# Artemarius/cuda-gaussian-splatting

Hardware: AMD Instinct MI355X
Metric: fwd+bwd Mpixels/s @1080p, 1M Gaussians, SH3 (higher is better)
Workload: dtype f32

## Files before the change

cuda-gaussian-splatting_amd/csrc/cugs_common.h:

```cpp
#pragma once

#include <hip/hip_runtime.h>
#include <stdint.h>

#include "../../include/cugs_hip.h"
#include "../../include/cugs_detmath.h"

#ifndef CUGS_BLOCK
#define CUGS_BLOCK 256
#endif
#define CUGS_WAVE 64

#define CUGS_RETURN_IF_HIP(expr)                    \
    do {                                            \
        hipError_t _e = (expr);                     \
        if (_e != hipSuccess) return (int)_e;       \
    } while (0)

#define CUGS_LAUNCH_CHECK() CUGS_RETURN_IF_HIP(hipGetLastError())

static inline bool cugs_aligned16(const void* p) { return (reinterpret_cast<uintptr_t>(p) & 15u) == 0; }

typedef float cugs_v4f __attribute__((ext_vector_type(4)));
typedef float cugs_v2f __attribute__((ext_vector_type(2)));
// ... 7 lines not shown
    __builtin_nontemporal_store(t, reinterpret_cast<cugs_v4f*>(p));
}
__device__ __forceinline__ void cugs_stnt(float* p, float v) { __builtin_nontemporal_store(v, p); }

struct CamArgs {
    float view[16];
    float fx, fy, cx, cy;
    int width, height;
    float cc[3];
    float log_mod;
};

static inline CamArgs cugs_make_cam_args(const cugs_camera* c, float scale_modifier) {
    CamArgs a;
    for (int i = 0; i < 16; ++i) a.view[i] = c->view[i];
    a.fx = c->fx; a.fy = c->fy; a.cx = c->cx; a.cy = c->cy;
    a.width = c->width; a.height = c->height;
    a.cc[0] = c->cam_center[0]; a.cc[1] = c->cam_center[1]; a.cc[2] = c->cam_center[2];
    a.log_mod = logf(scale_modifier + 1e-8f);
    return a;
}

int cugs_sort_key_slots(void* workspace, size_t bytes, int64_t n, int width, int height, uint32_t** keys, int4** rect,
                        uint32_t** prect, uint32_t** range_flag, uint32_t** zero, uint32_t* nzero)
    __attribute__((visibility("hidden")));

__device__ __forceinline__ unsigned cugs_xcd_remap(unsigned bid, unsigned nwg) {
    unsigned xcd = bid & 7u, q = nwg >> 3, r = nwg & 7u;
    unsigned base = (xcd < r) ? xcd * (q + 1u) : r * (q + 1u) + (xcd - r) * q;
    return base + (bid >> 3);
}

#ifndef CUGS_ROW_GROUP
#define CUGS_ROW_GROUP 2
#endif
__device__ __forceinline__ unsigned cugs_blend_tile(unsigned bid, unsigned ntx, unsigned nty) {
    const unsigned lin = cugs_xcd_remap(bid, ntx * nty);
#if CUGS_ROW_GROUP == 0
    return lin;
#else
    constexpr unsigned G = CUGS_ROW_GROUP;
    unsigned row = lin / ntx;
    const unsigned col = lin - row * ntx;
    const unsigned nunits = (nty + G - 1u) / G;
    unsigned c = 0, urow = row;
#pragma unroll
    for (unsigned k = 0; k < 7u; ++k) {
// ... 10 lines not shown
```

cuda-gaussian-splatting_amd/csrc/cugs_gaussian_math.h:

```cpp
#pragma once

#include "cugs_common.h"

struct V3 { float x, y, z; };
struct Sym2 { float a, b, c; };
struct Sym3 { float xx, xy, xz, yy, yz, zz; };
struct M3 { float m00, m01, m02, m10, m11, m12, m20, m21, m22; };
struct M23 { float r0x, r0y, r0z, r1x, r1y, r1z; };

struct GradMoments { float m1x, m1y, m2xx, m2xy, m2yy; };
struct Grad2D { float mx, my, a, b, c; };
__device__ __forceinline__ Grad2D grads_from_moments(const GradMoments& m, float a, float b, float c) {
    Grad2D g;
    g.mx = a * m.m1x + b * m.m1y;
    g.my = b * m.m1x + c * m.m1y;
    g.a = -0.5f * m.m2xx;
    g.b = -m.m2xy;
    g.c = -0.5f * m.m2yy;
    return g;
}

__device__ __forceinline__ M3 view_rotation(const CamArgs& c) {
    return M3{c.view[0], c.view[1], c.view[2], c.view[4], c.view[5], c.view[6],
              c.view[8], c.view[9], c.view[10]};
// ... 150 lines not shown
    *out_of_range = false;
    if (three_pass) {
        const uint32_t off = key - CUGS_DEPTH_KEY_BASE;
        const bool emits = tiles > 0 && w > 0;
        *out_of_range = emits && !(off >= 1u && off < CUGS_DEPTH_KEY_SPAN);
        key = emits ? min(off, CUGS_DEPTH_KEY_SPAN - 1u) : 0u;
    }
    return SortRecord{key, make_int4(x0, y0, w | (h << 16), tiles > 0 ? tiles : 0)};
}

constexpr int CUGS_PRECT_MAX_TILES = 127;
__host__ __device__ inline bool cugs_prect_packable(int ntx, int nty) { return ntx <= CUGS_PRECT_MAX_TILES && nty <= CUGS_PRECT_MAX_TILES; }
__device__ __forceinline__ uint32_t pack_rect(int4 r) {
    const int w = r.z & 0xFFFF, h = r.z >> 16;
    if (w == 0) return 0x80000000u | (uint32_t)r.w;
    return (uint32_t)r.x | ((uint32_t)r.y << 7) | ((uint32_t)w << 14) | ((uint32_t)h << 21);
}
__device__ __forceinline__ int4 unpack_rect(uint32_t v) {
    if (v & 0x80000000u) return make_int4(0, 0, 0, (int)(v & 0x7FFFFFFFu));
    const int x0 = (int)(v & 127u), y0 = (int)((v >> 7) & 127u), w = (int)((v >> 14) & 127u), h = (int)((v >> 21) & 127u);
    return make_int4(x0, y0, w | (h << 16), w * h);
}

__device__ __forceinline__ V3 view_direction(V3 p, const CamArgs& c) {
    float dx = p.x - c.cc[0], dy = p.y - c.cc[1], dz = p.z - c.cc[2];
    float nrm = fmaxf(sqrtf(dx * dx + dy * dy + dz * dz), 1e-8f);
    return V3{dx / nrm, dy / nrm, dz / nrm};
}

__device__ __forceinline__ void sh_basis(int degree, V3 d, float (&Y)[16]) {
    const float x = d.x, y = d.y, z = d.z;
    Y[0] = 0.28209479177387814f;
    if (degree >= 1) {
        Y[1] = -0.4886025119029199f * y;
        Y[2] = 0.4886025119029199f * z;
        Y[3] = -0.4886025119029199f * x;
    }
    if (degree >= 2) {
        const float xx = x * x, yy = y * y, zz = z * z;
        Y[4] = 1.0925484305920792f * (x * y);
        Y[5] = 1.0925484305920792f * (y * z);
        Y[6] = 0.31539156525252005f * (2 * zz - xx - yy);
        Y[7] = 1.0925484305920792f * (x * z);
        Y[8] = 0.5462742152960396f * (xx - yy);
    }
    if (degree >= 3) {
// ... 58 lines not shown
```

cuda-gaussian-splatting_amd/csrc/project_forward.hip:

```cpp
#include "cugs_gaussian_math.h"

namespace {

template <int C>
struct ShTile {
    static constexpr int ROW = 3 * C;
    static constexpr int LROW = (ROW % 2 == 0) ? ROW + 1 : ROW;
};

template <int C, bool ALIGNED>
__device__ __forceinline__ void stage_sh_rows(const float* __restrict__ sh, int64_t base, int count,
                                              float* s_sh) {
    constexpr int ROW = ShTile<C>::ROW, LROW = ShTile<C>::LROW;
    const float* src = sh + base * ROW;
    const int total = count * ROW;
    const int tid = threadIdx.x;
    if (ALIGNED && count == CUGS_BLOCK) {
        constexpr int TOTAL4 = CUGS_BLOCK * ROW / 4, PER = (TOTAL4 + CUGS_BLOCK - 1) / CUGS_BLOCK;
        const float4* src4 = reinterpret_cast<const float4*>(src);
        float4 v[PER];
#pragma unroll
        for (int i = 0; i < PER; ++i) {
            const int e4 = tid + i * CUGS_BLOCK;
            v[i] = (e4 < TOTAL4) ? cugs_ldnt(src4 + e4) : make_float4(0.f, 0.f, 0.f, 0.f);
// ... 23 lines not shown
#pragma unroll
            for (int k = 0; k < 4; ++k) {
                s_sh[row * LROW + col] = vals[k];
                if (++col == ROW) { col = 0; ++row; }
            }
        }
        for (int e = (total4 << 2) + tid; e < total; e += CUGS_BLOCK) {
            int row = e / ROW, col = e - row * ROW;
            s_sh[row * LROW + col] = src[e];
        }
    } else {
        for (int e = tid; e < total; e += CUGS_BLOCK) {
            int row = e / ROW, col = e - row * ROW;
            s_sh[row * LROW + col] = src[e];
        }
    }
}

struct ProjPtrs {
    const float* positions; const float* rotations; const float* scales; const float* opacities;
    const float* sh;
    float* means_2d; float* depths; float* cov_2d_inv; int32_t* radii; int32_t* tiles_touched;
    float* opacities_act; float* rgb; float* packed; uint8_t* colour_gate;
    uint32_t* sort_keys; int4* sort_rect; uint32_t* sort_prect; uint32_t* sort_range_flag;
    uint32_t* sort_zero; uint32_t sort_nzero;
};

template <int C, bool ALIGNED, int PART>
__global__ __launch_bounds__(CUGS_BLOCK) void k_project_forward(int64_t n, int degree, CamArgs cam,
                                                                ProjPtrs p) {
    constexpr int LROW = ShTile<C>::LROW;
    constexpr int OUT_F = 6 * CUGS_BLOCK + CUGS_PACKED_STRIDE * CUGS_BLOCK;
    constexpr int SH_F = (PART == 1) ? 0 : CUGS_BLOCK * LROW;
    __shared__ __attribute__((aligned(16))) float s_sh[SH_F > OUT_F ? SH_F : OUT_F];

    const int64_t base = (int64_t)blockIdx.x * CUGS_BLOCK;
    const int count = (int)min((int64_t)CUGS_BLOCK, n - base);
    for (uint32_t z = blockIdx.x * CUGS_BLOCK + threadIdx.x; z < p.sort_nzero; z += gridDim.x * CUGS_BLOCK) p.sort_zero[z] = 0u;
    const int64_t idx = base + threadIdx.x;
    const bool live = idx < n;
    const int64_t ld = live ? idx : (n - 1);
    const V3 pos{cugs_ldnt(p.positions + ld * 3 + 0), cugs_ldnt(p.positions + ld * 3 + 1), cugs_ldnt(p.positions + ld * 3 + 2)};
    float in_opa = 0.0f, in_s0 = 0.0f, in_s1 = 0.0f, in_s2 = 0.0f;
    float4 q = make_float4(1.0f, 0.0f, 0.0f, 0.0f);
    {
        in_opa = cugs_ldnt(p.opacities + ld);
        in_s0 = cugs_ldnt(p.scales + ld * 3 + 0); in_s1 = cugs_ldnt(p.scales + ld * 3 + 1); in_s2 = cugs_ldnt(p.scales + ld * 3 + 2);
// ... 46 lines not shown
        const Sym3 S = gram(scale_columns(qr.R, s));
        const Jac J = jacobian(t, cam.fx, cam.fy);
        const Sym2 cov = screen_covariance(project_matrix_full(J, W), S);
        Sym2 inv_c;
        const float det = invert_sym2(cov, inv_c);
        if (det > 0.0f) {
            inv = inv_c;
            int r = splat_radius(cov);
            if (r > 0) {
                r = min(r, max(cam.width, cam.height));
                radius = r;
                const int ntx = (cam.width + CUGS_TILE - 1) / CUGS_TILE;
                const int nty = (cam.height + CUGS_TILE - 1) / CUGS_TILE;
                tr = tile_rect_of(mx, my, r, cam.width, cam.height, ntx, nty);
                tiles = max((tr.x1 - tr.x0) * (tr.y1 - tr.y0), 0);
            }
        }
    }

    p.depths[idx] = depth;
    p.radii[idx] = radius;
    p.tiles_touched[idx] = tiles;
    p.opacities_act[idx] = opa;
    if (p.sort_keys) {
        bool bad;
        const SortRecord rec = sort_record_of(depth, tiles, radius, tr, true, &bad);
        if (bad) atomicOr(p.sort_range_flag, 1u);
        p.sort_keys[idx] = rec.key;
        if (p.sort_prect) p.sort_prect[idx] = pack_rect(rec.rect);
        else p.sort_rect[idx] = rec.rect;
    }
    if (ALIGNED && count == CUGS_BLOCK && p.packed) {
        reinterpret_cast<float2*>(p.means_2d)[idx] = make_float2(mx, my);
        if constexpr (PART == 0) __syncthreads();
        float* s_rgb = s_sh;
        float* s_cov = s_sh + 3 * CUGS_BLOCK;
        float4* s_pk = reinterpret_cast<float4*>(s_sh + 6 * CUGS_BLOCK);
        const int t = threadIdx.x;
        s_rgb[t * 3 + 0] = col[0]; s_rgb[t * 3 + 1] = col[1]; s_rgb[t * 3 + 2] = col[2];
        s_cov[t * 3 + 0] = inv.a; s_cov[t * 3 + 1] = inv.b; s_cov[t * 3 + 2] = inv.c;
        const float tau = (opa >= (1.0f / 255.0f)) ? logf(255.0f * opa) : -1.0f;
        s_pk[t * 3 + 0] = make_float4(mx, my, inv.a, inv.b);
        s_pk[t * 3 + 1] = make_float4(inv.c, opa, tau, 0.0f);
        s_pk[t * 3 + 2] = make_float4(col[0], 0.0f, col[1], col[2]);
        __syncthreads();
        if (t < 3 * CUGS_BLOCK / 4) {
            if constexpr (PART == 0) reinterpret_cast<float4*>(p.rgb + base * 3)[t] = reinterpret_cast<const float4*>(s_rgb)[t];
            reinterpret_cast<float4*>(p.cov_2d_inv + base * 3)[t] = reinterpret_cast<const float4*>(s_cov)[t];
        }
        float4* g_pk = reinterpret_cast<float4*>(p.packed + base * CUGS_PACKED_STRIDE);
        if constexpr (PART == 0) {
#pragma unroll
            for (int k = 0; k < 3; ++k) g_pk[t + k * CUGS_BLOCK] = s_pk[t + k * CUGS_BLOCK];
// ... 174 lines not shown
                                    const float* positions, const float* rotations,
                                    const float* scales, const float* opacities,
                                    const float* sh_coeffs, const cugs_camera* camera_host,
                                    float scale_modifier, float* means_2d, float* depths,
                                    float* cov_2d_inv, int32_t* radii, int32_t* tiles_touched,
                                    float* opacities_act, float* rgb, float* packed, uint8_t* colour_gate,
                                    void* sort_workspace, size_t sort_workspace_bytes, void* stream) {
    if (n < 0 || !camera_host) return CUGS_EINVAL;
    if (active_degree < 0 || active_degree > 3) return CUGS_EINVAL;
    if ((active_degree + 1) * (active_degree + 1) > num_coeffs) return CUGS_EINVAL;
    if (num_coeffs != 1 && num_coeffs != 4 && num_coeffs != 9 && num_coeffs != 16) return CUGS_EINVAL;
    if (n == 0) return 0;
    if (!positions || !rotations || !scales || !opacities || !sh_coeffs || !means_2d || !depths ||
        !cov_2d_inv || !radii || !tiles_touched || !opacities_act || !rgb)
        return CUGS_EINVAL;
    if (packed && !cugs_aligned16(packed)) return CUGS_EALIGN;
    if (n > (int64_t)2147483647) return CUGS_EOVERFLOW;

    const CamArgs cam = cugs_make_cam_args(camera_host, scale_modifier);
    ProjPtrs p{positions, rotations, scales, opacities, sh_coeffs, means_2d, depths, cov_2d_inv,
               radii, tiles_touched, opacities_act, rgb, packed, colour_gate, nullptr, nullptr, nullptr, nullptr, nullptr, 0u};
    if (sort_workspace) {
        int rc = cugs_sort_key_slots(sort_workspace, sort_workspace_bytes, n, camera_host->width, camera_host->height,
                                     &p.sort_keys, &p.sort_rect, &p.sort_prect, &p.sort_range_flag, &p.sort_zero, &p.sort_nzero);
        if (rc) return rc;
    }
    const bool aligned = cugs_aligned16(sh_coeffs) && cugs_aligned16(rotations) && cugs_aligned16(rgb) &&
                         cugs_aligned16(cov_2d_inv) && (reinterpret_cast<uintptr_t>(means_2d) & 7u) == 0;
    hipStream_t st = static_cast<hipStream_t>(stream);
    switch (num_coeffs) {
        case 1: return launch_project<1>(n, active_degree, cam, p, aligned, st);
        case 4: return launch_project<4>(n, active_degree, cam, p, aligned, st);
        case 9: return launch_project<9>(n, active_degree, cam, p, aligned, st);
        default: return launch_project<16>(n, active_degree, cam, p, aligned, st);
    }
}
}

extern "C" int cugs_project_forward(int64_t n, int num_coeffs, int active_degree,
                                    const float* positions, const float* rotations,
                                    const float* scales, const float* opacities,
                                    const float* sh_coeffs, const cugs_camera* camera_host,
                                    float scale_modifier, float* means_2d, float* depths,
                                    float* cov_2d_inv, int32_t* radii, int32_t* tiles_touched,
                                    float* opacities_act, float* rgb, float* packed, uint8_t* colour_gate,
                                    void* stream) {
    return project_forward_impl(n, num_coeffs, active_degree, positions, rotations, scales, opacities, sh_coeffs,
// ... 13 lines not shown
    return project_forward_impl(n, num_coeffs, active_degree, positions, rotations, scales, opacities, sh_coeffs,
                                camera_host, scale_modifier, means_2d, depths, cov_2d_inv, radii, tiles_touched,
                                opacities_act, rgb, packed, colour_gate, sort_workspace, sort_workspace_bytes, stream);
}

extern "C" int cugs_project_forward_geometry(int64_t n, const float* positions, const float* rotations,
                                             const float* scales, const float* opacities,
                                             const cugs_camera* camera_host, float scale_modifier, float* means_2d,
                                             float* depths, float* cov_2d_inv, int32_t* radii, int32_t* tiles_touched,
                                             float* opacities_act, float* packed, void* sort_workspace,
                                             size_t sort_workspace_bytes, void* stream) {
    if (n < 0 || !camera_host) return CUGS_EINVAL;
    if (n == 0) return 0;
    if (!positions || !rotations || !scales || !opacities || !means_2d || !depths || !cov_2d_inv || !radii ||
        !tiles_touched || !opacities_act)
        return CUGS_EINVAL;
    if (packed && !cugs_aligned16(packed)) return CUGS_EALIGN;
    if (n > (int64_t)2147483647) return CUGS_EOVERFLOW;
    const CamArgs cam = cugs_make_cam_args(camera_host, scale_modifier);
    ProjPtrs p{positions, rotations, scales, opacities, nullptr, means_2d, depths, cov_2d_inv, radii, tiles_touched,
               opacities_act, nullptr, packed, nullptr, nullptr, nullptr, nullptr, nullptr, nullptr, 0u};
    if (sort_workspace) {
        int rc = cugs_sort_key_slots(sort_workspace, sort_workspace_bytes, n, camera_host->width, camera_host->height,
                                     &p.sort_keys, &p.sort_rect, &p.sort_prect, &p.sort_range_flag, &p.sort_zero, &p.sort_nzero);
        if (rc) return rc;
    }
    const bool aligned = cugs_aligned16(rotations) && cugs_aligned16(cov_2d_inv) &&
                         (reinterpret_cast<uintptr_t>(means_2d) & 7u) == 0;
    return launch_project<1, 1>(n, 0, cam, p, aligned, static_cast<hipStream_t>(stream));
}

extern "C" int cugs_project_forward_colour(int64_t n, int num_coeffs, int active_degree, const float* positions,
                                           const float* sh_coeffs, const cugs_camera* camera_host, float* rgb,
                                           float* packed, uint8_t* colour_gate, void* stream) {
    if (n < 0 || !camera_host) return CUGS_EINVAL;
    if (active_degree < 0 || active_degree > 3) return CUGS_EINVAL;
    if ((active_degree + 1) * (active_degree + 1) > num_coeffs) return CUGS_EINVAL;
    if (num_coeffs != 1 && num_coeffs != 4 && num_coeffs != 9 && num_coeffs != 16) return CUGS_EINVAL;
    if (n == 0) return 0;
    if (!positions || !sh_coeffs || !rgb) return CUGS_EINVAL;
    if (packed && !cugs_aligned16(packed)) return CUGS_EALIGN;
    if (n > (int64_t)2147483647) return CUGS_EOVERFLOW;
    const CamArgs cam = cugs_make_cam_args(camera_host, 1.0f);
    ProjPtrs p{positions, nullptr, nullptr, nullptr, sh_coeffs, nullptr, nullptr, nullptr, nullptr, nullptr, nullptr, rgb,
               packed, colour_gate, nullptr, nullptr, nullptr, nullptr, nullptr, 0u};
    const bool aligned = cugs_aligned16(sh_coeffs) && cugs_aligned16(rgb);
    hipStream_t st = static_cast<hipStream_t>(stream);
// ... 47 lines not shown
```

cuda-gaussian-splatting_amd/csrc/sort.hip:

```cpp
#include "sort_workspace.h"
#include "sort_radix.h"
#include "sort_emit.h"
#include "sort_tile_order.h"
#include "sort_bin.h"

namespace {

int queue_count(const SortPlan& plan, const SortWsN& ws, const float* means_2d, const float* depths, const int32_t* radii,
                const int32_t* tiles_touched, hipStream_t st, unsigned long long* total_mapped) {
    const uint32_t un = plan.n;
    const int ntx = plan.ntx, nty = plan.nty;
    const bool narrow = plan.depth == DepthRoute::Narrow, direct = plan.route == PairRoute::Direct;
    uint32_t* const range_flag = &ws.ctl->range_flag;
    uint32_t* const q12 = &ws.ctl->q12_count;
    const uint32_t* const ridden = plan.riding ? ws.prect[1] : nullptr;
    int rc;
    if (plan.keys == KeySource::Built) {
        hipLaunchKernelGGL(k_depth_keys_rect, dim3(nblocks_for(un, CUGS_BLOCK)), dim3(CUGS_BLOCK), 0, st, un, depths,
                           means_2d, radii, tiles_touched, plan.width, plan.height, ntx, nty, ws.dkey[narrow ? 0 : 1], ws.rect[0],
                           narrow ? range_flag : static_cast<uint32_t*>(nullptr), ws.sup, plan.depth_clear);
        CUGS_LAUNCH_CHECK();
    }
    uint32_t* sp[SUP_TABLES];
    for (int t = 0; t < SUP_TABLES; ++t) sp[t] = ws.sup + (size_t)t * plan.depth_table;
    if (narrow) {
        uint32_t* const* pr = ws.prect;
        const bool riding = plan.riding;
        if ((rc = radix_pass<uint32_t, true, 1024, CHUNK_DEPTH, RADIX_DEPTH>(ws.dkey[0], nullptr, un, nullptr, 0, DEPTH_BITS, ws.hist, sp[0], ws.tot, ws.dkey[1], ws.dval[1], nullptr, st, riding ? pr[0] : nullptr, pr[1]))) return rc;
        if ((rc = radix_pass<uint32_t, false, 1024, CHUNK_DEPTH, RADIX_DEPTH>(ws.dkey[1], ws.dval[1], un, nullptr, DEPTH_BITS, DEPTH_BITS, ws.hist, sp[1], ws.tot, ws.dkey[0], ws.dval[0], nullptr, st, riding ? pr[1] : nullptr, pr[0]))) return rc;
        if ((rc = radix_pass<uint32_t, false, 1024, CHUNK_DEPTH, RADIX_DEPTH>(ws.dkey[0], ws.dval[0], un, nullptr, 2 * DEPTH_BITS, DEPTH_BITS, ws.hist, sp[2], ws.tot, ws.dkey[1], ws.dval[1], direct ? q12 : nullptr, st, riding ? pr[0] : nullptr, pr[1]))) return rc;
    } else {
        if ((rc = radix_pass<uint32_t, true, 1024, CHUNK_MIN>(ws.dkey[1], nullptr, un, nullptr, 0, 8, ws.hist, sp[0], ws.tot, ws.dkey[0], ws.dval[0], nullptr, st))) return rc;
        if ((rc = radix_pass<uint32_t, false, 1024, CHUNK_MIN>(ws.dkey[0], ws.dval[0], un, nullptr, 8, 8, ws.hist, sp[1], ws.tot, ws.dkey[1], ws.dval[1], nullptr, st))) return rc;
        if ((rc = radix_pass<uint32_t, false, 1024, CHUNK_MIN>(ws.dkey[1], ws.dval[1], un, nullptr, 16, 8, ws.hist, sp[2], ws.tot, ws.dkey[0], ws.dval[0], nullptr, st))) return rc;
        if ((rc = radix_pass<uint32_t, false, 1024, CHUNK_MIN>(ws.dkey[0], ws.dval[0], un, nullptr, 24, 8, ws.hist, sp[3], ws.tot, ws.dkey[1], ws.dval[1], nullptr, st))) return rc;
    }
    if (direct) {
        const uint32_t tiles = (uint32_t)plan.tiles, rows = bin_rows(un);
        hipLaunchKernelGGL(k_bin_count, dim3(rows), dim3(BIN_NT), 0, st, un, BIN_GROUP, ws.dval[1], ws.rect[0], ridden,
                           plan.riding ? static_cast<uint32_t*>(nullptr) : ws.prect[1], (uint32_t)ntx, (uint32_t)nty, ws.bin_table, q12,
                           ws.bin_win);
        CUGS_LAUNCH_CHECK();
        hipLaunchKernelGGL(k_bin_scan, dim3((tiles + CUGS_WAVE - 1) / CUGS_WAVE), dim3(BIN_NT), 0, st, rows, tiles, ws.bin_table,
                           ws.bin_ttot, ws.bin_tpre, ws.bin_csum, q12, range_flag, &ws.ctl->snap_q12,
                           bin_windows(ntx, nty) <= BIN_WINDOWS_MAX ? ws.bin_win : nullptr,
                           (uint32_t)ntx, bin_window_cols(ntx), bin_window_groups(ntx));
        CUGS_LAUNCH_CHECK();
        return 0;
    }
    const uint32_t nfill = nblocks_for(un, FILL_CHUNK);
    hipLaunchKernelGGL(k_fill_blocksums, dim3(nfill), dim3(CUGS_BLOCK), 0, st, un, ws.dval[1], ws.rect[0], ws.rect[1],
                       ws.blocksum, ridden);
    CUGS_LAUNCH_CHECK();
// ... 74 lines not shown
        const int shift = p * per;
        const int b = (bits - shift) < per ? (bits - shift) : per;
        uint32_t* vout = (p == npass - 1) ? vals_final : tv[cur ^ 1];
        rc = radix_pass<K, false, 512, CHUNK_PAIR>(tk[cur], tv[cur], up, dev_count, shift, b, wp.hist, wp.sup + sup_off[p], ws.tot,
                                                   tk[cur ^ 1], vout, p == 0 ? ctl : nullptr, st);
        if (rc) return rc;
        cur ^= 1;
    }
    hipLaunchKernelGGL((k_tile_ranges<K, false>), dim3(nblocks_for(up, CUGS_BLOCK * 8)), dim3(CUGS_BLOCK), 0, st, up, dev_count, tk[cur],
                       (uint32_t)ntx, values_sorted, depths, tile_ranges, keys_sorted, ctl + 1);
    CUGS_LAUNCH_CHECK();
    return 0;
}

template <typename... A>
int sort_pairs_dispatch(const SortPlan& plan, A... args) {
    if (plan.wide_ids) return sort_pairs_typed<uint32_t>(plan, args...);
    return sort_pairs_typed<uint16_t>(plan, args...);
}

}

int cugs_sort_key_slots(void* workspace, size_t bytes, int64_t n, int width, int height, uint32_t** keys, int4** rect,
                        uint32_t** prect, uint32_t** range_flag, uint32_t** zero, uint32_t* nzero) {
    if (!workspace || n < 0 || n > 2147483647ll || width < 0 || height < 0) return CUGS_EINVAL;
    if ((width + CUGS_TILE - 1) / CUGS_TILE > 32767 || (height + CUGS_TILE - 1) / CUGS_TILE > 32767) return CUGS_EOVERFLOW;
    SortWsN ws = carve_n(workspace, n);
    if (bytes < ws.bytes) return CUGS_EWORKSPACE;
    const SortPlan plan = make_sort_plan(n, width, height, 0, KeySource::Prekeyed, DepthRoute::Narrow, PairCount::Predicted);
    *keys = ws.dkey[0];
    *rect = plan.riding ? nullptr : ws.rect[0];
    *prect = plan.riding ? ws.prect[0] : nullptr;
    *range_flag = &ws.ctl->range_flag;
    *zero = ws.sup;
    *nzero = plan.depth_clear;
    return 0;
}

extern "C" size_t cugs_sort_workspace_bytes(int64_t n) {
    if (n < 0) return 0;
    return carve_n(nullptr, n).bytes;
}

extern "C" size_t cugs_sort_pair_workspace_bytes(int64_t total_pairs) {
    if (total_pairs < 0) return 0;
    return carve_p(nullptr, total_pairs).bytes;
}

namespace {
int sort_count_pairs_impl(int64_t n, const float* means_2d, const float* depths,
                                     const int32_t* radii, const int32_t* tiles_touched, int width,
                                     int height, void* workspace, size_t workspace_bytes,
                                     int64_t* total_pairs_host, void* stream, DepthRoute depth) {
    if (n < 0 || width < 0 || height < 0 || !total_pairs_host) return CUGS_EINVAL;
    *total_pairs_host = 0;
// ... 220 lines not shown
```

cuda-gaussian-splatting_amd/csrc/sort_radix.h:

```cpp
#pragma once

#include "sort_workspace.h"

namespace {

__device__ __forceinline__ uint32_t wave_inclusive_scan(uint32_t v) {
    const int lane = threadIdx.x & 63;
#pragma unroll
    for (int d = 1; d < 64; d <<= 1) {
        uint32_t t = __shfl_up(v, d);
        if (lane >= d) v += t;
    }
    return v;
}

template <int NW = 4>
__device__ __forceinline__ uint32_t block_exclusive_scan(uint32_t v, uint32_t* s_tmp, uint32_t* total) {
    const int lane = threadIdx.x & 63, wave = threadIdx.x >> 6;
    uint32_t inc = wave_inclusive_scan(v);
    if (lane == 63) s_tmp[wave] = inc;
    __syncthreads();
    uint32_t base = 0, sum = 0;
#pragma unroll
    for (int w = 0; w < NW; ++w) {
// ... 249 lines not shown
__global__ __launch_bounds__(CUGS_BLOCK) void k_probe_lds_order(uint32_t* __restrict__ violations) {
    __shared__ uint32_t cnt[4][RADIX];
    const uint32_t wave = threadIdx.x >> 6, lane = threadIdx.x & 63, set = blockIdx.x;
    for (uint32_t i = threadIdx.x; i < 4 * RADIX; i += CUGS_BLOCK) (&cnt[0][0])[i] = 0;
    __syncthreads();
    uint32_t d[8], got[8];
#pragma unroll
    for (int r = 0; r < 8; ++r) d[r] = probe_digit(set, wave, r, lane);
#pragma unroll
    for (int r = 0; r < 8; ++r) got[r] = atomicAdd(&cnt[wave][d[r]], 1u);
    uint32_t bad = 0;
    for (int r = 0; r < 8; ++r) {
        uint32_t expect = 0;
        for (int rr = 0; rr <= r; ++rr)
            for (uint32_t l = 0; l < 64u && !(rr == r && l >= lane); ++l) expect += probe_digit(set, wave, rr, l) == d[r];
        bad += expect != got[r];
    }
    if (bad) atomicAdd(violations, bad);
}
#endif

template <typename K, bool IOTA, int NT, int CHUNK, int RDX = RADIX>
int radix_pass(const K* kin, const uint32_t* vin, uint32_t count, const unsigned long long* dev_count, int shift, int bits,
               uint32_t* hist, uint32_t* sup, uint32_t* tot, K* kout, uint32_t* vout, uint32_t* ctl, hipStream_t st,
               const uint32_t* v2in = nullptr, uint32_t* v2out = nullptr) {
    const uint32_t nblk = nblocks_for(count, CHUNK);
    const uint32_t sb = sup_block(nblk);
    static_assert(NT % RDX == 0, "whole thread groups per digit");
    if (!scan_free(nblk, (uint32_t)NT >> bits)) sup = nullptr;
    hipLaunchKernelGGL((k_radix_hist<K, NT, CHUNK, RDX>), dim3(nblk), dim3(NT), 0, st, kin, count, dev_count, shift,
                       (1u << bits) - 1u, hist, nblk, ctl, sup, sb);
    CUGS_LAUNCH_CHECK();
    if (!sup) {
        hipLaunchKernelGGL(k_radix_scan_rows, dim3(RDX), dim3(CUGS_BLOCK), 0, st, hist, hist, nblk, tot);
        CUGS_LAUNCH_CHECK();
    }
    if constexpr (RDX == RADIX_DEPTH) {
        if (v2in)
            hipLaunchKernelGGL((k_radix_scatter<K, IOTA, DEPTH_BITS, NT, false, CHUNK, RDX, true>), dim3(nblk), dim3(NT), 0, st, kin,
                               vin, count, dev_count, shift, 0u, hist, sup, sb, tot, nblk, kout, vout, v2in, v2out);
        else
            hipLaunchKernelGGL((k_radix_scatter<K, IOTA, DEPTH_BITS, NT, false, CHUNK, RDX>), dim3(nblk), dim3(NT), 0, st, kin, vin, count,
                               dev_count, shift, 0u, hist, sup, sb, tot, nblk, kout, vout);
        CUGS_LAUNCH_CHECK();
        return 0;
    }
    if (v2in) return CUGS_EINVAL;
#ifdef CUGS_DEV
    if (rank_mode() == 1) {
        hipLaunchKernelGGL((k_radix_scatter<K, IOTA, 8, NT, true, CHUNK>), dim3(nblk), dim3(NT), 0, st, kin, vin, count, dev_count,
                           shift, (1u << bits) - 1u, hist, sup, sb, tot, nblk, kout, vout);
        CUGS_LAUNCH_CHECK();
        return 0;
    }
#endif
#define CUGS_SCATTER(NB)                                                                                          \
    hipLaunchKernelGGL((k_radix_scatter<K, IOTA, NB, NT, false, CHUNK>), dim3(nblk), dim3(NT), 0, st, kin, vin, count, dev_count, \
                       shift, 0u, hist, sup, sb, tot, nblk, kout, vout)
    switch (bits) {
        case 1: CUGS_SCATTER(1); break;
        case 2: CUGS_SCATTER(2); break;
        case 3: CUGS_SCATTER(3); break;
        case 4: CUGS_SCATTER(4); break;
        case 5: CUGS_SCATTER(5); break;
        case 6: CUGS_SCATTER(6); break;
        case 7: CUGS_SCATTER(7); break;
        default: CUGS_SCATTER(8); break;
    }
#undef CUGS_SCATTER
    CUGS_LAUNCH_CHECK();
// ... 5 lines not shown
```

cuda-gaussian-splatting_amd/csrc/sort_workspace.h:

```cpp
#pragma once

#include "cugs_gaussian_math.h"

#include <atomic>
#include <cstddef>

namespace {

constexpr int RADIX = 256;
constexpr int RADIX_DEPTH = 512, DEPTH_BITS = CUGS_DEPTH_BITS;
constexpr int IPT = 16;
constexpr int CHUNK_MIN = CUGS_BLOCK * IPT;
constexpr int CHUNK_DEPTH = 4096;
static_assert(CHUNK_DEPTH <= CHUNK_MIN && CHUNK_MIN % CHUNK_DEPTH == 0, "the histogram buffers are carved for CHUNK_DEPTH blocks");
constexpr int CHUNK_PAIR = CHUNK_MIN;
constexpr int FILL_CHUNK = CUGS_BLOCK;
constexpr int COL_WAVES = 16;
constexpr int COL_CHUNK = COL_WAVES * CUGS_WAVE;
static_assert(COL_CHUNK % FILL_CHUNK == 0, "whole FILL_CHUNK blocks per column workgroup");

inline size_t align_up(size_t v, size_t a) { return (v + a - 1) / a * a; }
inline uint32_t nblocks_for(int64_t count, int chunk) { return (uint32_t)((count + chunk - 1) / chunk); }

constexpr int SUP_TABLES = 4;
constexpr uint32_t SCANFREE_MAX_BLOCKS = 4096u, SCANFREE_MAX_LOADS = 26u;
inline uint32_t sup_block(uint32_t nblk) { return nblk <= 512u ? 16u : 64u; }
inline bool scan_free(uint32_t nblk, uint32_t grp) {
    const uint32_t sb = sup_block(nblk);
    return nblk <= SCANFREE_MAX_BLOCKS && ((nblk + sb - 1u) / sb + sb) <= SCANFREE_MAX_LOADS * grp;
}
inline uint32_t sup_rows(uint32_t nblk, uint32_t grp) { return scan_free(nblk, grp) ? (nblk + sup_block(nblk) - 1u) / sup_block(nblk) : 0u; }
inline uint32_t sup_rows_bound(uint32_t nblk) { return (nblk < SCANFREE_MAX_BLOCKS ? nblk : SCANFREE_MAX_BLOCKS) / 16u + 4u; }
inline uint32_t sup_used(uint32_t nblk, int rdx, uint32_t grp) { return (uint32_t)rdx * sup_rows(nblk, grp); }

constexpr int BIN_TILES_CAP = 10240;
constexpr uint32_t BIN_GROUP = 4096u, BIN_ROWS_MAX = 512u;
constexpr uint32_t BIN_WINDOWS_MAX = 64u;
inline bool bin_route_n(int64_t n) { return n <= (int64_t)BIN_GROUP * BIN_ROWS_MAX; }
// ... 60 lines not shown
    Carver c{static_cast<char*>(base)};
    SortWsN w;
    w.ctl = reinterpret_cast<SortCtl*>(c.take<unsigned long long>(SORT_CTL_WORDS));
    for (int i = 0; i < 2; ++i) w.dkey[i] = c.take<uint32_t>((size_t)n);
    for (int i = 0; i < 2; ++i) w.dval[i] = c.take<uint32_t>((size_t)n);
    for (int i = 0; i < 2; ++i) w.rect[i] = c.take<int4>((size_t)n);
    for (int i = 0; i < 2; ++i) w.prect[i] = c.take<uint32_t>((size_t)n);
    w.tot = c.take<uint32_t>(RADIX_DEPTH);
    w.blocksum = c.take<uint32_t>((size_t)nblocks_for(n, FILL_CHUNK) + 2);
    w.hist = c.take<uint32_t>((size_t)RADIX_DEPTH * (nblocks_for(n, CHUNK_DEPTH) + 1));
    w.sup_entries = (uint32_t)RADIX_DEPTH * sup_rows_bound(nblocks_for(n, CHUNK_DEPTH));
    w.sup = c.take<uint32_t>((size_t)SUP_TABLES * w.sup_entries);
    w.colhist = c.take<uint32_t>((size_t)RADIX * (nblocks_for(n, COL_CHUNK) + 1));
    w.colscan = c.take<uint32_t>((size_t)RADIX * (nblocks_for(n, COL_CHUNK) + 1));
    w.bin_table = c.take<uint32_t>((size_t)bin_table_rows(n) * BIN_TILES_CAP);
    w.bin_ttot = c.take<uint32_t>(BIN_TILES_CAP);
    w.bin_tpre = c.take<uint32_t>(BIN_TILES_CAP);
    w.bin_csum = c.take<uint32_t>(BIN_TILES_CAP / 64 + 4);
    w.bin_win = c.take<uint32_t>(BIN_WINDOWS_MAX);
    w.bin_tbase = c.take<uint32_t>(BIN_TILES_CAP + 1);
    w.bytes = c.off;
    return w;
}
SortWsP carve_p(void* base, int64_t pairs) {
    Carver c{static_cast<char*>(base)};
    SortWsP w;
    for (int i = 0; i < 2; ++i) w.ptile[i] = c.take<uint32_t>((size_t)pairs);
    for (int i = 0; i < 2; ++i) w.pidx[i] = c.take<uint32_t>((size_t)pairs);
    w.hist = c.take<uint32_t>((size_t)RADIX * (nblocks_for(pairs, CHUNK_MIN) + 1));
    w.sup_entries = (uint32_t)RADIX * sup_rows_bound(nblocks_for(pairs, CHUNK_MIN));
    w.sup = c.take<uint32_t>((size_t)SUP_TABLES * w.sup_entries);
    w.bytes = c.off;
    return w;
}

#ifdef CUGS_DEV
std::atomic<int> g_rank_mode{-1};
std::atomic<int> g_direct_route{1};
std::atomic<int> g_col_min_ratio{13};
inline int rank_mode() { return g_rank_mode.load(std::memory_order_relaxed); }
inline bool direct_route_enabled() { return g_direct_route.load(std::memory_order_relaxed) != 0; }
inline uint32_t column_min_ratio() { return (uint32_t)g_col_min_ratio.load(std::memory_order_relaxed); }
#else
constexpr int rank_mode() { return 0; }
constexpr bool direct_route_enabled() { return true; }
constexpr uint32_t column_min_ratio() { return 13u; }
// ... 26 lines not shown
    uint32_t depth_clear;
    bool riding;
    PairCount count;
    PairRoute route;
    bool wide_ids;
    int pair_passes, pair_bits;
    bool staged;
};

inline SortPlan make_sort_plan(int64_t n, int width, int height, int64_t pairs, KeySource keys, DepthRoute depth, PairCount count) {
    SortPlan p{};
    p.n = (uint32_t)n; p.pairs = (uint32_t)pairs;
    p.width = width; p.height = height;
    p.ntx = (width + CUGS_TILE - 1) / CUGS_TILE; p.nty = (height + CUGS_TILE - 1) / CUGS_TILE;
    p.tiles = p.ntx * p.nty;
    p.depth = depth;
    p.keys = depth == DepthRoute::Narrow ? keys : KeySource::Built;
    const bool narrow = depth == DepthRoute::Narrow;
    p.depth_passes = narrow ? 3 : 4;
    p.depth_nblk = nblocks_for(n, narrow ? CHUNK_DEPTH : CHUNK_MIN);
    p.depth_grp = 1024u >> (narrow ? DEPTH_BITS : 8);
    p.depth_table = sup_used(p.depth_nblk, narrow ? RADIX_DEPTH : RADIX, p.depth_grp);
    p.depth_clear = (uint32_t)p.depth_passes * p.depth_table;
    p.riding = p.keys == KeySource::Prekeyed && cugs_prect_packable(p.ntx, p.nty) && nblocks_for(n, CHUNK_MIN) <= 256u;
    p.count = count;
    p.wide_ids = tile_bits(p.tiles) > 16;
    if (count == PairCount::Predicted && p.keys == KeySource::Prekeyed && bin_route(p.ntx, p.nty) && bin_route_n(n) &&
        pairs < (int64_t(1) << 30) && direct_route_enabled()) {
        p.route = PairRoute::Direct;
        p.staged = (unsigned long long)p.pairs >= (unsigned long long)BIN_STAGE_RATIO * p.n;
    } else if (column_path(p.ntx, p.nty) && column_path_pays(p.n, p.pairs)) {
        p.route = PairRoute::Column;
        p.pair_passes = 1;
        p.pair_bits = tile_bits(p.nty);
    } else {
        p.route = PairRoute::Radix;
        const int bits = tile_bits(p.tiles);
        p.pair_passes = (bits + 7) / 8;
        p.pair_bits = (bits + p.pair_passes - 1) / p.pair_passes;
    }
    return p;
}

}
```

Before: 2719.

## Pack depth key and tile rectangle into one 64-bit record for riding depth sort

Projection now writes the depth key and packed tile rectangle as a single 64-bit word, and a new three-pass depth sort moves these packed records, folding the Gaussian index into the upper bits after the first pass. This replaces the previous radix passes that carried separate key, value and rectangle arrays, cutting the number of separate streams each scatter reads and writes. It adds custom histogram and scatter kernels with 64-bit shared staging, which raises LDS use per block, and limits the riding path to counts whose indices fit in 20 bits.

After: 2739, median of 6. About the same (+0.7%).

```diff
diff --git a/cuda-gaussian-splatting_amd/csrc/cugs_common.h b/cuda-gaussian-splatting_amd/csrc/cugs_common.h
--- a/cuda-gaussian-splatting_amd/csrc/cugs_common.h
+++ b/cuda-gaussian-splatting_amd/csrc/cugs_common.h
@@ -53,7 +53,7 @@
 }
 
 int cugs_sort_key_slots(void* workspace, size_t bytes, int64_t n, int width, int height, uint32_t** keys, int4** rect,
-                        uint32_t** prect, uint32_t** range_flag, uint32_t** zero, uint32_t* nzero)
+                        unsigned long long** packed, uint32_t** range_flag, uint32_t** zero, uint32_t* nzero)
     __attribute__((visibility("hidden")));
 
 __device__ __forceinline__ unsigned cugs_xcd_remap(unsigned bid, unsigned nwg) {
diff --git a/cuda-gaussian-splatting_amd/csrc/cugs_gaussian_math.h b/cuda-gaussian-splatting_amd/csrc/cugs_gaussian_math.h
--- a/cuda-gaussian-splatting_amd/csrc/cugs_gaussian_math.h
+++ b/cuda-gaussian-splatting_amd/csrc/cugs_gaussian_math.h
@@ -196,6 +196,10 @@
     return make_int4(x0, y0, w | (h << 16), w * h);
 }
 
+__device__ __forceinline__ unsigned long long pack_depth_record(uint32_t key, uint32_t prect) {
+    return ((unsigned long long)key << 32) | prect;
+}
+
 __device__ __forceinline__ V3 view_direction(V3 p, const CamArgs& c) {
     float dx = p.x - c.cc[0], dy = p.y - c.cc[1], dz = p.z - c.cc[2];
     float nrm = fmaxf(sqrtf(dx * dx + dy * dy + dz * dz), 1e-8f);
diff --git a/cuda-gaussian-splatting_amd/csrc/project_forward.hip b/cuda-gaussian-splatting_amd/csrc/project_forward.hip
--- a/cuda-gaussian-splatting_amd/csrc/project_forward.hip
+++ b/cuda-gaussian-splatting_amd/csrc/project_forward.hip
@@ -69,7 +69,7 @@
     const float* sh;
     float* means_2d; float* depths; float* cov_2d_inv; int32_t* radii; int32_t* tiles_touched;
     float* opacities_act; float* rgb; float* packed; uint8_t* colour_gate;
-    uint32_t* sort_keys; int4* sort_rect; uint32_t* sort_prect; uint32_t* sort_range_flag;
+    uint32_t* sort_keys; int4* sort_rect; unsigned long long* sort_packed; uint32_t* sort_range_flag;
     uint32_t* sort_zero; uint32_t sort_nzero;
 };
 
@@ -162,13 +162,16 @@
     p.radii[idx] = radius;
     p.tiles_touched[idx] = tiles;
     p.opacities_act[idx] = opa;
-    if (p.sort_keys) {
+    if (p.sort_range_flag) {
         bool bad;
         const SortRecord rec = sort_record_of(depth, tiles, radius, tr, true, &bad);
         if (bad) atomicOr(p.sort_range_flag, 1u);
-        p.sort_keys[idx] = rec.key;
-        if (p.sort_prect) p.sort_prect[idx] = pack_rect(rec.rect);
-        else p.sort_rect[idx] = rec.rect;
+        if (p.sort_packed) {
+            p.sort_packed[idx] = pack_depth_record(rec.key, pack_rect(rec.rect));
+        } else {
+            p.sort_keys[idx] = rec.key;
+            p.sort_rect[idx] = rec.rect;
+        }
     }
     if (ALIGNED && count == CUGS_BLOCK && p.packed) {
         reinterpret_cast<float2*>(p.means_2d)[idx] = make_float2(mx, my);
@@ -389,7 +392,7 @@
                radii, tiles_touched, opacities_act, rgb, packed, colour_gate, nullptr, nullptr, nullptr, nullptr, nullptr, 0u};
     if (sort_workspace) {
         int rc = cugs_sort_key_slots(sort_workspace, sort_workspace_bytes, n, camera_host->width, camera_host->height,
-                                     &p.sort_keys, &p.sort_rect, &p.sort_prect, &p.sort_range_flag, &p.sort_zero, &p.sort_nzero);
+                                     &p.sort_keys, &p.sort_rect, &p.sort_packed, &p.sort_range_flag, &p.sort_zero, &p.sort_nzero);
         if (rc) return rc;
     }
     const bool aligned = cugs_aligned16(sh_coeffs) && cugs_aligned16(rotations) && cugs_aligned16(rgb) &&
@@ -449,7 +452,7 @@
                opacities_act, nullptr, packed, nullptr, nullptr, nullptr, nullptr, nullptr, nullptr, 0u};
     if (sort_workspace) {
         int rc = cugs_sort_key_slots(sort_workspace, sort_workspace_bytes, n, camera_host->width, camera_host->height,
-                                     &p.sort_keys, &p.sort_rect, &p.sort_prect, &p.sort_range_flag, &p.sort_zero, &p.sort_nzero);
+                                     &p.sort_keys, &p.sort_rect, &p.sort_packed, &p.sort_range_flag, &p.sort_zero, &p.sort_nzero);
         if (rc) return rc;
     }
     const bool aligned = cugs_aligned16(rotations) && cugs_aligned16(cov_2d_inv) &&
diff --git a/cuda-gaussian-splatting_amd/csrc/sort.hip b/cuda-gaussian-splatting_amd/csrc/sort.hip
--- a/cuda-gaussian-splatting_amd/csrc/sort.hip
+++ b/cuda-gaussian-splatting_amd/csrc/sort.hip
@@ -1,5 +1,6 @@
 #include "sort_workspace.h"
 #include "sort_radix.h"
+#include "sort_depth_pack.h"
 #include "sort_emit.h"
 #include "sort_tile_order.h"
 #include "sort_bin.h"
@@ -24,11 +25,17 @@
     uint32_t* sp[SUP_TABLES];
     for (int t = 0; t < SUP_TABLES; ++t) sp[t] = ws.sup + (size_t)t * plan.depth_table;
     if (narrow) {
-        uint32_t* const* pr = ws.prect;
-        const bool riding = plan.riding;
-        if ((rc = radix_pass<uint32_t, true, 1024, CHUNK_DEPTH, RADIX_DEPTH>(ws.dkey[0], nullptr, un, nullptr, 0, DEPTH_BITS, ws.hist, sp[0], ws.tot, ws.dkey[1], ws.dval[1], nullptr, st, riding ? pr[0] : nullptr, pr[1]))) return rc;
-        if ((rc = radix_pass<uint32_t, false, 1024, CHUNK_DEPTH, RADIX_DEPTH>(ws.dkey[1], ws.dval[1], un, nullptr, DEPTH_BITS, DEPTH_BITS, ws.hist, sp[1], ws.tot, ws.dkey[0], ws.dval[0], nullptr, st, riding ? pr[1] : nullptr, pr[0]))) return rc;
-        if ((rc = radix_pass<uint32_t, false, 1024, CHUNK_DEPTH, RADIX_DEPTH>(ws.dkey[0], ws.dval[0], un, nullptr, 2 * DEPTH_BITS, DEPTH_BITS, ws.hist, sp[2], ws.tot, ws.dkey[1], ws.dval[1], direct ? q12 : nullptr, st, riding ? pr[0] : nullptr, pr[1]))) return rc;
+        if (plan.riding) {
+            uint64_t* const a = packed_over_dkey(ws);
+            uint64_t* const c = packed_over_prect(ws);
+            if ((rc = depth_pack_pass<1>(a, nullptr, un, ws.hist, sp[0], c, ws.dval[0], nullptr, nullptr, st))) return rc;
+            if ((rc = depth_pack_pass<2>(c, ws.dval[0], un, ws.hist, sp[1], a, nullptr, nullptr, nullptr, st))) return rc;
+            if ((rc = depth_pack_pass<3>(a, nullptr, un, ws.hist, sp[2], nullptr, ws.dval[1], ws.prect[1], direct ? q12 : nullptr, st))) return rc;
+        } else {
+            if ((rc = radix_pass<uint32_t, true, 1024, CHUNK_DEPTH, RADIX_DEPTH>(ws.dkey[0], nullptr, un, nullptr, 0, DEPTH_BITS, ws.hist, sp[0], ws.tot, ws.dkey[1], ws.dval[1], nullptr, st))) return rc;
+            if ((rc = radix_pass<uint32_t, false, 1024, CHUNK_DEPTH, RADIX_DEPTH>(ws.dkey[1], ws.dval[1], un, nullptr, DEPTH_BITS, DEPTH_BITS, ws.hist, sp[1], ws.tot, ws.dkey[0], ws.dval[0], nullptr, st))) return rc;
+            if ((rc = radix_pass<uint32_t, false, 1024, CHUNK_DEPTH, RADIX_DEPTH>(ws.dkey[0], ws.dval[0], un, nullptr, 2 * DEPTH_BITS, DEPTH_BITS, ws.hist, sp[2], ws.tot, ws.dkey[1], ws.dval[1], direct ? q12 : nullptr, st))) return rc;
+        }
     } else {
         if ((rc = radix_pass<uint32_t, true, 1024, CHUNK_MIN>(ws.dkey[1], nullptr, un, nullptr, 0, 8, ws.hist, sp[0], ws.tot, ws.dkey[0], ws.dval[0], nullptr, st))) return rc;
         if ((rc = radix_pass<uint32_t, false, 1024, CHUNK_MIN>(ws.dkey[0], ws.dval[0], un, nullptr, 8, 8, ws.hist, sp[1], ws.tot, ws.dkey[1], ws.dval[1], nullptr, st))) return rc;
@@ -149,15 +156,15 @@
 }
 
 int cugs_sort_key_slots(void* workspace, size_t bytes, int64_t n, int width, int height, uint32_t** keys, int4** rect,
-                        uint32_t** prect, uint32_t** range_flag, uint32_t** zero, uint32_t* nzero) {
+                        unsigned long long** packed, uint32_t** range_flag, uint32_t** zero, uint32_t* nzero) {
     if (!workspace || n < 0 || n > 2147483647ll || width < 0 || height < 0) return CUGS_EINVAL;
     if ((width + CUGS_TILE - 1) / CUGS_TILE > 32767 || (height + CUGS_TILE - 1) / CUGS_TILE > 32767) return CUGS_EOVERFLOW;
     SortWsN ws = carve_n(workspace, n);
     if (bytes < ws.bytes) return CUGS_EWORKSPACE;
     const SortPlan plan = make_sort_plan(n, width, height, 0, KeySource::Prekeyed, DepthRoute::Narrow, PairCount::Predicted);
-    *keys = ws.dkey[0];
+    *keys = plan.riding ? nullptr : ws.dkey[0];
     *rect = plan.riding ? nullptr : ws.rect[0];
-    *prect = plan.riding ? ws.prect[0] : nullptr;
+    *packed = plan.riding ? reinterpret_cast<unsigned long long*>(packed_over_dkey(ws)) : nullptr;
     *range_flag = &ws.ctl->range_flag;
     *zero = ws.sup;
     *nzero = plan.depth_clear;
diff --git a/cuda-gaussian-splatting_amd/csrc/sort_depth_pack.h b/cuda-gaussian-splatting_amd/csrc/sort_depth_pack.h
--- /dev/null
+++ b/cuda-gaussian-splatting_amd/csrc/sort_depth_pack.h
@@ -0,0 +1,197 @@
+#pragma once
+
+#include "sort_radix.h"
+
+namespace {
+
+constexpr int DEPTH_PACK_RECT_BITS = 32;
+constexpr int DEPTH_PACK_KEY_BITS = 3 * DEPTH_BITS;
+static_assert(DEPTH_BITS + DEPTH_PACK_IDX_BITS + DEPTH_PACK_RECT_BITS <= 64, "R2: last digit, index and rectangle in one word");
+static_assert(DEPTH_PACK_KEY_BITS + DEPTH_PACK_RECT_BITS <= 64, "P0: whole key and rectangle in one word");
+static_assert((1u << DEPTH_PACK_KEY_BITS) == CUGS_DEPTH_KEY_SPAN, "sort_record_of clamps the key to the bits packed here");
+static_assert(CHUNK_DEPTH == CHUNK_MIN, "RIDING_MAX_BLOCKS counts the workgroups of these passes");
+
+constexpr int depth_pack_digit_bit(int pass) { return pass == 3 ? DEPTH_PACK_RECT_BITS + DEPTH_PACK_IDX_BITS : DEPTH_PACK_RECT_BITS; }
+
+template <int PASS>
+__device__ __forceinline__ uint32_t depth_pack_digit(uint32_t hi) {
+    constexpr int BIT = depth_pack_digit_bit(PASS) - 32;
+    static_assert(BIT >= 0 && BIT + DEPTH_BITS <= 32, "the digit lies in the upper dword");
+    return (hi >> BIT) & (uint32_t)(RADIX_DEPTH - 1);
+}
+
+template <int PASS>
+__global__ __launch_bounds__(1024) void k_depth_pack_hist(const uint64_t* __restrict__ recs, uint32_t count,
+                                                          uint32_t* __restrict__ hist, uint32_t* __restrict__ ctl,
+                                                          uint32_t* __restrict__ sup, uint32_t sb) {
+    constexpr int NT = 1024, CHUNK = CHUNK_DEPTH, RDX = RADIX_DEPTH;
+    constexpr int PER = CHUNK / NT;
+    static_assert(PER % 2 == 0, "whole 16-byte loads per thread");
+    __shared__ uint32_t s_cnt[RDX];
+    if (threadIdx.x < RDX) s_cnt[threadIdx.x] = 0;
+    if (ctl && blockIdx.x == 0 && threadIdx.x == 0) { ctl[1] = ctl[0]; ctl[0] = 0u; }
+    __syncthreads();
+    const uint32_t bbase = blockIdx.x * CHUNK;
+    if (bbase + CHUNK <= count) {
+        const uint4* src = reinterpret_cast<const uint4*>(recs + bbase + threadIdx.x * PER);
+        uint32_t hi[PER];
+#pragma unroll
+        for (int v = 0; v < PER / 2; ++v) {
+            const uint4 q = src[v];
+            hi[2 * v] = q.y; hi[2 * v + 1] = q.w;
+        }
+#pragma unroll
+        for (int c = 0; c < PER; ++c) atomicAdd(&s_cnt[depth_pack_digit<PASS>(hi[c])], 1u);
+    } else {
+        for (uint32_t i = bbase + threadIdx.x; i < count; i += NT)
+            atomicAdd(&s_cnt[depth_pack_digit<PASS>((uint32_t)(recs[i] >> 32))], 1u);
+    }
+    __syncthreads();
+    if (threadIdx.x < RDX) {
+        const uint32_t c = s_cnt[threadIdx.x];
+        hist[(size_t)blockIdx.x * RDX + threadIdx.x] = c;
+        if (c) atomicAdd(&sup[(size_t)(blockIdx.x / sb) * RDX + threadIdx.x], c);
+    }
+}
+
+template <int PASS>
+__global__ __launch_bounds__(1024) void k_depth_pack_scatter(
+    const uint64_t* __restrict__ rec_in, const uint32_t* __restrict__ idx_in, uint32_t count,
+    const uint32_t* __restrict__ hist, const uint32_t* __restrict__ sup, uint32_t sb, uint32_t nblk,
+    uint64_t* __restrict__ rec_out, uint32_t* __restrict__ idx_out, uint32_t* __restrict__ prect_out) {
+    static_assert(PASS >= 1 && PASS <= 3, "three passes");
+    constexpr int NT = 1024, CHUNK = CHUNK_DEPTH, RDX = RADIX_DEPTH, NB = DEPTH_BITS;
+    constexpr bool IDX = PASS != 3;
+    if (blockIdx.x * CHUNK >= count) return;
+    constexpr int NW = NT / CUGS_WAVE;
+    constexpr int PER = CHUNK / NT;
+    constexpr int SLICE = CUGS_WAVE * PER;
+    static_assert(NT >= RDX && (1 << NB) == RDX && NT % RDX == 0, "whole thread groups per digit");
+    __shared__ uint32_t s_lbase[NW][RDX];
+    __shared__ uint32_t s_lstart[RDX];
+    __shared__ uint32_t s_gbase[RDX];
+    __shared__ uint64_t s_rec[CHUNK];
+    __shared__ uint32_t s_idx[IDX ? CHUNK : 1];
+    __shared__ uint32_t s_tmp[NW];
+    const uint32_t tid = threadIdx.x, wave = tid >> 6, lane = tid & 63;
+    const uint32_t bbase = blockIdx.x * CHUNK;
+    const uint32_t wbase = bbase + wave * SLICE;
+    const uint32_t count_blk = min((uint32_t)CHUNK, count - bbase);
+
+    constexpr int GRP = NT / RDX;
+    uint32_t pre = 0u, totd = 0u;
+    {
+        const uint32_t d = tid % RDX, part = tid / RDX;
+        const uint32_t mysb = blockIdx.x / sb, nsb = (nblk + sb - 1u) / sb;
+#pragma unroll 4
+        for (uint32_t r = part; r < nsb; r += GRP) {
+            const uint32_t v = sup[(size_t)r * RDX + d];
+            totd += v;
+            pre += (r < mysb) ? v : 0u;
+        }
+#pragma unroll 4
+        for (uint32_t b2 = mysb * sb + part; b2 < blockIdx.x; b2 += GRP) pre += hist[(size_t)b2 * RDX + d];
+    }
+
+    for (uint32_t e = tid; e < NW * RDX; e += NT) (&s_lbase[0][0])[e] = 0;
+    if (tid < RDX) { s_gbase[tid] = 0u; s_lstart[tid] = 0u; }
+    __syncthreads();
+    if (pre) atomicAdd(&s_gbase[tid % RDX], pre);
+    if (totd) atomicAdd(&s_lstart[tid % RDX], totd);
+
+    uint64_t rec[PER];
+    uint32_t idx[IDX ? PER : 1];
+#pragma unroll
+    for (int r = 0; r < PER; ++r) {
+        const uint32_t i = wbase + r * CUGS_WAVE + lane;
+        const bool ok = i < count;
+        rec[r] = ok ? __builtin_nontemporal_load(rec_in + i) : ~0ull;
+        if constexpr (PASS == 1) idx[r] = i;
+        if constexpr (PASS == 2) idx[r] = ok ? __builtin_nontemporal_load(idx_in + i) : 0u;
+        if (ok) atomicAdd(&s_lbase[wave][depth_pack_digit<PASS>((uint32_t)(rec[r] >> 32))], 1u);
+    }
+    __syncthreads();
+
+    {
+        const bool dig = tid < RDX;
+        uint32_t cnt = 0;
+        if (dig) {
+#pragma unroll
+            for (int w = 0; w < NW; ++w) cnt += s_lbase[w][tid];
+        }
+        const uint32_t before = dig ? s_gbase[tid] : 0u;
+        const uint32_t dig_base = block_exclusive_scan<NW>(dig ? s_lstart[tid] : 0u, s_tmp, nullptr);
+        const uint32_t lstart = block_exclusive_scan<NW>(cnt, s_tmp, nullptr);
+        if (dig) {
+            s_gbase[tid] = dig_base + before;
+            s_lstart[tid] = lstart;
+            uint32_t run = lstart;
+#pragma unroll
+            for (int w = 0; w < NW; ++w) {
+                const uint32_t c = s_lbase[w][tid];
+                s_lbase[w][tid] = run;
+                run += c;
+            }
+        }
+    }
+    __syncthreads();
+
+    const unsigned long long lt_mask = (1ull << lane) - 1ull;
+#pragma unroll
+    for (int r = 0; r < PER; ++r) {
+        const uint32_t i = wbase + r * CUGS_WAVE + lane;
+        const bool ok = i < count;
+        const uint32_t d = depth_pack_digit<PASS>((uint32_t)(rec[r] >> 32));
+        unsigned long long peers = __ballot(ok);
+#pragma unroll
+        for (int b = 0; b < NB; ++b) {
+            const bool bit = (d >> b) & 1u;
+            const unsigned long long m = __ballot(bit);
+            peers &= bit ? m : ~m;
+        }
+        if (ok) {
+            const uint32_t base = s_lbase[wave][d];
+            const uint32_t pos = base + __popcll(peers & lt_mask);
+            s_rec[pos] = rec[r];
+            if constexpr (IDX) s_idx[pos] = idx[r];
+            if ((peers >> lane) == 1ull) s_lbase[wave][d] = base + __popcll(peers);
+        }
+    }
+    __syncthreads();
+
+#pragma unroll
+    for (int r = 0; r < PER; ++r) {
+        const uint32_t j = r * NT + tid;
+        if (j < count_blk) {
+            const uint64_t in = s_rec[j];
+            const uint32_t hi = (uint32_t)(in >> 32), lo = (uint32_t)in;
+            const uint32_t d = depth_pack_digit<PASS>(hi);
+            const uint32_t dst = s_gbase[d] + (j - s_lstart[d]);
+            if constexpr (PASS == 1) {
+                rec_out[dst] = ((uint64_t)(hi >> NB) << 32) | lo;
+                idx_out[dst] = s_idx[j];
+            } else if constexpr (PASS == 2) {
+                rec_out[dst] = ((uint64_t)(((hi >> NB) << DEPTH_PACK_IDX_BITS) | s_idx[j]) << 32) | lo;
+            } else {
+                idx_out[dst] = hi & ((1u << DEPTH_PACK_IDX_BITS) - 1u);
+                prect_out[dst] = lo;
+            }
+        }
+    }
+}
+
+template <int PASS>
+int depth_pack_pass(const uint64_t* rec_in, const uint32_t* idx_in, uint32_t count, uint32_t* hist, uint32_t* sup,
+                    uint64_t* rec_out, uint32_t* idx_out, uint32_t* prect_out, uint32_t* ctl, hipStream_t st) {
+    const uint32_t nblk = nblocks_for(count, CHUNK_DEPTH);
+    const uint32_t sb = sup_block(nblk);
+    if (count > (1u << DEPTH_PACK_IDX_BITS) || !scan_free(nblk, 1024u >> DEPTH_BITS)) return CUGS_EINVAL;
+    hipLaunchKernelGGL((k_depth_pack_hist<PASS>), dim3(nblk), dim3(1024), 0, st, rec_in, count, hist, ctl, sup, sb);
+    CUGS_LAUNCH_CHECK();
+    hipLaunchKernelGGL((k_depth_pack_scatter<PASS>), dim3(nblk), dim3(1024), 0, st, rec_in, idx_in, count, hist, sup, sb, nblk,
+                       rec_out, idx_out, prect_out);
+    CUGS_LAUNCH_CHECK();
+    return 0;
+}
+
+}
diff --git a/cuda-gaussian-splatting_amd/csrc/sort_radix.h b/cuda-gaussian-splatting_amd/csrc/sort_radix.h
--- a/cuda-gaussian-splatting_amd/csrc/sort_radix.h
+++ b/cuda-gaussian-splatting_amd/csrc/sort_radix.h
@@ -295,8 +295,7 @@
 
 template <typename K, bool IOTA, int NT, int CHUNK, int RDX = RADIX>
 int radix_pass(const K* kin, const uint32_t* vin, uint32_t count, const unsigned long long* dev_count, int shift, int bits,
-               uint32_t* hist, uint32_t* sup, uint32_t* tot, K* kout, uint32_t* vout, uint32_t* ctl, hipStream_t st,
-               const uint32_t* v2in = nullptr, uint32_t* v2out = nullptr) {
+               uint32_t* hist, uint32_t* sup, uint32_t* tot, K* kout, uint32_t* vout, uint32_t* ctl, hipStream_t st) {
     const uint32_t nblk = nblocks_for(count, CHUNK);
     const uint32_t sb = sup_block(nblk);
     static_assert(NT % RDX == 0, "whole thread groups per digit");
@@ -309,16 +308,11 @@
         CUGS_LAUNCH_CHECK();
     }
     if constexpr (RDX == RADIX_DEPTH) {
-        if (v2in)
-            hipLaunchKernelGGL((k_radix_scatter<K, IOTA, DEPTH_BITS, NT, false, CHUNK, RDX, true>), dim3(nblk), dim3(NT), 0, st, kin,
-                               vin, count, dev_count, shift, 0u, hist, sup, sb, tot, nblk, kout, vout, v2in, v2out);
-        else
-            hipLaunchKernelGGL((k_radix_scatter<K, IOTA, DEPTH_BITS, NT, false, CHUNK, RDX>), dim3(nblk), dim3(NT), 0, st, kin, vin, count,
-                               dev_count, shift, 0u, hist, sup, sb, tot, nblk, kout, vout);
+        hipLaunchKernelGGL((k_radix_scatter<K, IOTA, DEPTH_BITS, NT, false, CHUNK, RDX>), dim3(nblk), dim3(NT), 0, st, kin, vin, count,
+                           dev_count, shift, 0u, hist, sup, sb, tot, nblk, kout, vout);
         CUGS_LAUNCH_CHECK();
         return 0;
     }
-    if (v2in) return CUGS_EINVAL;
 #ifdef CUGS_DEV
     if (rank_mode() == 1) {
         hipLaunchKernelGGL((k_radix_scatter<K, IOTA, 8, NT, true, CHUNK>), dim3(nblk), dim3(NT), 0, st, kin, vin, count, dev_count,
diff --git a/cuda-gaussian-splatting_amd/csrc/sort_workspace.h b/cuda-gaussian-splatting_amd/csrc/sort_workspace.h
--- a/cuda-gaussian-splatting_amd/csrc/sort_workspace.h
+++ b/cuda-gaussian-splatting_amd/csrc/sort_workspace.h
@@ -14,6 +14,9 @@
 constexpr int CHUNK_DEPTH = 4096;
 static_assert(CHUNK_DEPTH <= CHUNK_MIN && CHUNK_MIN % CHUNK_DEPTH == 0, "the histogram buffers are carved for CHUNK_DEPTH blocks");
 constexpr int CHUNK_PAIR = CHUNK_MIN;
+constexpr uint32_t RIDING_MAX_BLOCKS = 256u;
+constexpr int DEPTH_PACK_IDX_BITS = 20;
+static_assert((unsigned long long)RIDING_MAX_BLOCKS * CHUNK_MIN <= (1ull << DEPTH_PACK_IDX_BITS), "every index of a riding sort fits the packed record");
 constexpr int FILL_CHUNK = CUGS_BLOCK;
 constexpr int COL_WAVES = 16;
 constexpr int COL_CHUNK = COL_WAVES * CUGS_WAVE;
@@ -120,6 +123,8 @@
     w.bytes = c.off;
     return w;
 }
+inline uint64_t* packed_over_dkey(const SortWsN& w) { return reinterpret_cast<uint64_t*>(w.dkey[0]); }
+inline uint64_t* packed_over_prect(const SortWsN& w) { return reinterpret_cast<uint64_t*>(w.prect[0]); }
 SortWsP carve_p(void* base, int64_t pairs) {
     Carver c{static_cast<char*>(base)};
     SortWsP w;
@@ -192,7 +197,7 @@
     p.depth_grp = 1024u >> (narrow ? DEPTH_BITS : 8);
     p.depth_table = sup_used(p.depth_nblk, narrow ? RADIX_DEPTH : RADIX, p.depth_grp);
     p.depth_clear = (uint32_t)p.depth_passes * p.depth_table;
-    p.riding = p.keys == KeySource::Prekeyed && cugs_prect_packable(p.ntx, p.nty) && nblocks_for(n, CHUNK_MIN) <= 256u;
+    p.riding = p.keys == KeySource::Prekeyed && cugs_prect_packable(p.ntx, p.nty) && nblocks_for(n, CHUNK_MIN) <= RIDING_MAX_BLOCKS;
     p.count = count;
     p.wide_ids = tile_bits(p.tiles) > 16;
     if (count == PairCount::Predicted && p.keys == KeySource::Prekeyed && bin_route(p.ntx, p.nty) && bin_route_n(n) &&
```
